# ebanalyse/ebnerd-benchmark

Hardware: AMD Instinct MI355X
Metric: training impressions/sec (higher is better)
Workload: dtype f32

## Files before the change

### ebnerd-benchmark_amd/csrc/ebn_attpool.hip

```cpp
#include "ebn_common.h"
#include "ebn_reduce.h"

namespace {

constexpr int POOL_THREADS = 256;
constexpr int POOL_WAVES = POOL_THREADS / 64;
constexpr float KERAS_EPS = 1e-7f;

__global__ __launch_bounds__(POOL_THREADS) void attpool_fwd_kernel(float* __restrict__ U,
                                                                    const float* __restrict__ b,
                                                                    const float* __restrict__ q,
                                                                    const float* __restrict__ X,
                                                                    float* __restrict__ out,
                                                                    float* __restrict__ w, int L, int E, int A) {
  extern __shared__ float sm[];
  const int64_t n = blockIdx.x;
  const int tid = threadIdx.x, lane = tid & 63, wave = tid >> 6;
  for (int l = wave; l < L; l += POOL_WAVES) {
    float* urow = U + (n * L + l) * A;
    float part = 0.f;
    for (int k = lane; k < A; k += 64) {
      const float u = tanhf(urow[k] + b[k]);
      urow[k] = u;
      part = fmaf(u, q[k], part);
// ... 40 lines not shown
    part = ebn_wave_sum(part);
    if (lane == 0) sm[l] = part;
  }
  __syncthreads();
  if (wave == 0) {
    float s = 0.f;
    for (int l = lane; l < L; l += 64) s = fmaf(w[n * L + l], sm[l], s);
    s = ebn_wave_sum(s);
    for (int l = lane; l < L; l += 64) de[n * L + l] = w[n * L + l] * (sm[l] - s);
  }
  if (dX == nullptr) return;
  for (int l = 0; l < L; ++l) {
    const float wl = w[n * L + l];
    float* dr = dX + (n * L + l) * E;
    for (int c = tid; c < E; c += POOL_THREADS) dr[c] = wl * g[c];
  }
}

constexpr int POOL_RB = 8;

__device__ __forceinline__ float4 ld4_clamped(const float* __restrict__ base, int64_t off, bool ok) {
  return *reinterpret_cast<const float4*>(base + (ok ? off : 0));
}
__device__ __forceinline__ float4 ld4_or_zero(const float* __restrict__ base, int64_t off, bool ok) {
  const float4 v = ld4_clamped(base, off, ok);
  float4 r;
  r.x = ok ? v.x : 0.f;
  r.y = ok ? v.y : 0.f;
  r.z = ok ? v.z : 0.f;
  r.w = ok ? v.w : 0.f;
  return r;
}

__global__ __launch_bounds__(POOL_THREADS) void attpool_fwd_vec_kernel(float* __restrict__ U,
                                                                        const float* __restrict__ b,
                                                                        const float* __restrict__ q,
                                                                        const float* __restrict__ X,
                                                                        float* __restrict__ out,
                                                                        float* __restrict__ w, int L, int E, int A) {
  extern __shared__ float sm[];
  __shared__ float4 part_acc[POOL_THREADS];
  const int64_t n = blockIdx.x;
  const int tid = threadIdx.x, lane = tid & 63, wave = tid >> 6;
  const int A4 = A >> 2, E4 = E >> 2;
  {
    const bool kok = lane < A4;
    const float4 bb = ld4_or_zero(b, lane * 4, kok), qq = ld4_or_zero(q, lane * 4, kok);
    for (int l0 = wave; l0 < L; l0 += POOL_WAVES * POOL_RB) {
      float4 u[POOL_RB];
#pragma unroll
      for (int j = 0; j < POOL_RB; ++j) {
        const int l = l0 + POOL_WAVES * j;
        u[j] = ld4_clamped(U, (n * L + l) * A + lane * 4, kok && l < L);
      }
#pragma unroll
      for (int j = 0; j < POOL_RB; ++j) {
        const int l = l0 + POOL_WAVES * j;
        if (l >= L) break;
        float4 t;
        t.x = tanhf(u[j].x + bb.x);
        t.y = tanhf(u[j].y + bb.y);
        t.z = tanhf(u[j].z + bb.z);
        t.w = tanhf(u[j].w + bb.w);
        if (kok) *reinterpret_cast<float4*>(U + (n * L + l) * A + lane * 4) = t;
        float part = kok ? fmaf(t.w, qq.w, fmaf(t.z, qq.z, fmaf(t.y, qq.y, t.x * qq.x))) : 0.f;
        part = ebn_wave_sum(part);
        if (lane == 0) sm[l] = part;
      }
    }
  }
  __syncthreads();
  if (wave == 0) {
    float s = 0.f;
    for (int l = lane; l < L; l += 64) {
      const float a = expf(sm[l]);
      sm[l] = a;
      s += a;
    }
    s = ebn_wave_sum(s) + KERAS_EPS;
    for (int l = lane; l < L; l += 64) {
      const float wl = sm[l] / s;
      sm[l] = wl;
      w[n * L + l] = wl;
    }
  }
  __syncthreads();
  const int NP = (E4 <= POOL_THREADS) ? POOL_THREADS / E4 : 1;
  for (int c0 = 0; c0 < E4; c0 += POOL_THREADS) {
    const int c4 = c0 + tid % ((E4 <= POOL_THREADS) ? E4 : POOL_THREADS);
    const int part = (E4 <= POOL_THREADS) ? tid / E4 : 0;
    const bool ok = c4 < E4 && part < NP;
    float4 acc = make_float4(0.f, 0.f, 0.f, 0.f);
    for (int l0 = part; l0 < L; l0 += NP * POOL_RB) {
      float4 x[POOL_RB];
#pragma unroll
      for (int j = 0; j < POOL_RB; ++j) {
        const int l = l0 + NP * j;
        x[j] = ld4_clamped(X, (n * L + l) * E + c4 * 4, ok && l < L);
      }
#pragma unroll
      for (int j = 0; j < POOL_RB; ++j) {
        const int l = l0 + NP * j;
        const float wl = (l < L) ? sm[l] : 0.f;
        acc.x = fmaf(wl, x[j].x, acc.x);
        acc.y = fmaf(wl, x[j].y, acc.y);
        acc.z = fmaf(wl, x[j].z, acc.z);
        acc.w = fmaf(wl, x[j].w, acc.w);
      }
    }
    if (NP > 1) {
      part_acc[tid] = acc;
      __syncthreads();
      if (part == 0 && ok) {
        for (int pp = 1; pp < NP; ++pp) {
          const float4 o = part_acc[pp * E4 + c4];
          acc.x += o.x;
          acc.y += o.y;
          acc.z += o.z;
          acc.w += o.w;
        }
      }
      __syncthreads();
    }
    if (part == 0 && ok) *reinterpret_cast<float4*>(out + n * E + c4 * 4) = acc;
  }
}

__global__ __launch_bounds__(POOL_THREADS) void attpool_bwd_pool_vec_kernel(const float* __restrict__ X,
                                                                             const float* __restrict__ w,
                                                                             const float* __restrict__ dout,
                                                                             float* __restrict__ dX,
                                                                             float* __restrict__ de, int L, int E,
                                                                             int write_dx) {
  extern __shared__ float sm[];
  const int64_t n = blockIdx.x;
  const int tid = threadIdx.x, lane = tid & 63, wave = tid >> 6;
  const int E4 = E >> 2;
  const float* g = dout + n * E;
  constexpr int VL = 4;
  float4 gg[VL];
#pragma unroll
  for (int v = 0; v < VL; ++v) gg[v] = ld4_or_zero(g, (lane + 64 * v) * 4, lane + 64 * v < E4);
  for (int l0 = wave; l0 < L; l0 += POOL_WAVES * POOL_RB) {
    float part[POOL_RB];
#pragma unroll
    for (int j = 0; j < POOL_RB; ++j) part[j] = 0.f;
#pragma unroll
    for (int v = 0; v < VL; ++v) {
      if (64 * v >= E4) break;
      float4 x[POOL_RB];
#pragma unroll
      for (int j = 0; j < POOL_RB; ++j) {
        const int l = l0 + POOL_WAVES * j;
        x[j] = ld4_clamped(X, (n * L + l) * E + (lane + 64 * v) * 4, l < L && lane + 64 * v < E4);
      }
#pragma unroll
      for (int j = 0; j < POOL_RB; ++j)
        part[j] = fmaf(gg[v].w, x[j].w, fmaf(gg[v].z, x[j].z, fmaf(gg[v].y, x[j].y, fmaf(gg[v].x, x[j].x, part[j]))));
    }
#pragma unroll
    for (int j = 0; j < POOL_RB; ++j) {
      const int l = l0 + POOL_WAVES * j;
      const float t = ebn_wave_sum(part[j]);
      if (lane == 0 && l < L) sm[l] = t;
    }
  }
  __syncthreads();
  if (wave == 0) {
    float s = 0.f;
    for (int l = lane; l < L; l += 64) s = fmaf(w[n * L + l], sm[l], s);
    s = ebn_wave_sum(s);
    for (int l = lane; l < L; l += 64) de[n * L + l] = w[n * L + l] * (sm[l] - s);
  }
  if (!write_dx) return;
  for (int c4 = tid; c4 < E4; c4 += POOL_THREADS) {
    const float4 gv = *reinterpret_cast<const float4*>(g + c4 * 4);
    for (int l = 0; l < L; ++l) {
      const float wl = w[n * L + l];
      *reinterpret_cast<float4*>(dX + (n * L + l) * E + c4 * 4) = make_float4(wl * gv.x, wl * gv.y, wl * gv.z, wl * gv.w);
    }
  }
}

__global__ __launch_bounds__(POOL_THREADS) void attpool_bwd_dpre_kernel(float* __restrict__ U,
                                                                         const float* __restrict__ q,
                                                                         const float* __restrict__ de,
                                                                         float* __restrict__ partials,
                                                                         int64_t R, int A, int64_t rpb) {
  const int64_t r0 = static_cast<int64_t>(blockIdx.x) * rpb;
  const int64_t r1 = (r0 + rpb < R) ? r0 + rpb : R;
  for (int k = threadIdx.x; k < A; k += POOL_THREADS) {
    const float qk = q[k];
    float dq = 0.f, db = 0.f;
    for (int64_t rb = r0; rb < r1; rb += 8) {
      float u[8], der[8];
#pragma unroll
      for (int j = 0; j < 8; ++j) {
        const int64_t r = (rb + j < r1) ? rb + j : r1 - 1;
        u[j] = U[r * A + k];
        der[j] = de[r];
      }
#pragma unroll
      for (int j = 0; j < 8; ++j) {
        if (rb + j >= r1) break;
        dq = fmaf(der[j], u[j], dq);
// ... 45 lines not shown
        *reinterpret_cast<float4*>(U + r * A + c4 * 4) = dp;
        db.x += dp.x;
        db.y += dp.y;
        db.z += dp.z;
        db.w += dp.w;
      }
    }
    *reinterpret_cast<float4*>(&sm[rs * A + c4 * 4]) = dq;
    *reinterpret_cast<float4*>(&sm[(RS + rs) * A + c4 * 4]) = db;
  }
  __syncthreads();
  for (int k = tid; k < A; k += POOL_THREADS) {
    float tq = 0.f, tb = 0.f;
    for (int i = 0; i < RS; ++i) {
      tq += sm[i * A + k];
      tb += sm[(RS + i) * A + k];
    }
    partials[(static_cast<int64_t>(blockIdx.x) * 2 + 0) * A + k] = tq;
    partials[(static_cast<int64_t>(blockIdx.x) * 2 + 1) * A + k] = tb;
  }
}

extern "C" int64_t ebn_attpool_partials_len(int64_t R, int32_t A) { return ebn_dim_ok(R, A) ? ebn_colred_blocks(R) * 2 * A : 0; }

extern "C" int ebn_attpool_fwd_f32(float* U, const float* b, const float* q, const float* X, float* out,
                                   float* w, int64_t n_seq, int32_t L, int32_t E, int32_t A,
                                   ebn_stream_t stream) {
  EBN_REQUIRE(U && b && q && X && out && w, EBN_ERR_BAD_ARG);
  EBN_REQUIRE(n_seq >= 0 && L > 0 && E > 0 && A > 0, EBN_ERR_BAD_ARG);
  EBN_REQUIRE(L <= 8192, EBN_ERR_UNSUPPORTED);
  if (n_seq == 0) return EBN_OK;
  const bool vec = (A % 4 == 0) && A <= 256 && (E % 4 == 0) && E <= 1024 && ebn_aligned16(U) && ebn_aligned16(b) &&
                   ebn_aligned16(q) && ebn_aligned16(X) && ebn_aligned16(out);
  if (vec)
    EBN_LAUNCH(attpool_fwd_vec_kernel, dim3(static_cast<unsigned>(n_seq)), dim3(POOL_THREADS),
                       L * sizeof(float), ebn_stream(stream), U, b, q, X, out, w, L, E, A);
  else
    EBN_LAUNCH(attpool_fwd_kernel, dim3(static_cast<unsigned>(n_seq)), dim3(POOL_THREADS),
                       L * sizeof(float), ebn_stream(stream), U, b, q, X, out, w, L, E, A);
  EBN_CHECK_LAUNCH();
  return EBN_OK;
}

extern "C" int ebn_attpool_bwd_pool_f32(const float* X, const float* w, const float* dout, float* dX,
                                        float* de, int64_t n_seq, int32_t L, int32_t E,
                                        ebn_stream_t stream) {
  EBN_REQUIRE(X && w && dout && de, EBN_ERR_BAD_ARG);
  EBN_REQUIRE(n_seq >= 0 && L > 0 && E > 0, EBN_ERR_BAD_ARG);
  EBN_REQUIRE(L <= 8192, EBN_ERR_UNSUPPORTED);
  if (n_seq == 0) return EBN_OK;
  const bool vec = (E % 4 == 0) && E <= 1024 && ebn_aligned16(X) && ebn_aligned16(dout) && ebn_aligned16(dX);
  if (vec)
    EBN_LAUNCH(attpool_bwd_pool_vec_kernel, dim3(static_cast<unsigned>(n_seq)), dim3(POOL_THREADS),
                       L * sizeof(float), ebn_stream(stream), X, w, dout, dX, de, L, E, dX != nullptr ? 1 : 0);
  else
    EBN_LAUNCH(attpool_bwd_pool_kernel, dim3(static_cast<unsigned>(n_seq)), dim3(POOL_THREADS),
                       L * sizeof(float), ebn_stream(stream), X, w, dout, dX, de, L, E);
  EBN_CHECK_LAUNCH();
  return EBN_OK;
}

extern "C" int ebn_attpool_bwd_dpre_f32(float* U, const float* q, const float* de, float* dq, float* db,
                                        float* partials, int64_t R, int32_t A, int32_t accumulate,
                                        ebn_stream_t stream) {
  EBN_REQUIRE(U && q && de && partials && ((dq != nullptr) == (db != nullptr)), EBN_ERR_BAD_ARG);
  EBN_REQUIRE(R >= 0 && A > 0, EBN_ERR_BAD_ARG);
  if (R == 0) return EBN_OK;
  const int64_t nb = ebn_colred_blocks(R);
  const int64_t rpb = ebn_ceil_div(R, nb);
  if ((A % 4) == 0 && A >= 4 && A <= 1024 && ebn_aligned16(U) && ebn_aligned16(q)) {
    const size_t lds = static_cast<size_t>(2) * (POOL_THREADS / (A / 4)) * A * sizeof(float);
    EBN_LAUNCH(attpool_bwd_dpre_vec_kernel, dim3(static_cast<unsigned>(nb)), dim3(POOL_THREADS), lds, ebn_stream(stream), U, q, de, partials,
                       R, A, rpb);
  } else {
    EBN_LAUNCH(attpool_bwd_dpre_kernel, dim3(static_cast<unsigned>(nb)), dim3(POOL_THREADS), 0,
                       ebn_stream(stream), U, q, de, partials, R, A, rpb);
  }
  EBN_CHECK_LAUNCH();
  if (dq == nullptr) return EBN_OK;
  ebn_reduce_partials(partials, nb, 2, A, 1.0f, dq, db, accumulate, nullptr, nullptr, ebn_stream(stream));
  EBN_CHECK_LAUNCH();
  return EBN_OK;
}
```

### ebnerd-benchmark_amd/csrc/ebn_gemm.hip

```cpp
#include <stdlib.h>

#include "ebn_common.h"
#include "ebn_finish.h"
#include "ebn_tn_finale.h"

typedef float ebn_f32x4 __attribute__((ext_vector_type(4)));
typedef int ebn_i32x4 __attribute__((ext_vector_type(4)));
__device__ ebn_f32x4 ebn_raw_buffer_load_x4(ebn_i32x4 rsrc, int voffset, int soffset, int aux) __asm("llvm.amdgcn.raw.buffer.load.v4f32");
__device__ void ebn_raw_buffer_load_lds(ebn_i32x4 rsrc, __attribute__((address_space(3))) void* lds, int size, int voffset,
                                        int soffset, int offset, int aux) __asm("llvm.amdgcn.raw.buffer.load.lds");

int ebn_gemm_direct_tn_slices(int64_t M, int64_t N, int64_t K);
int ebn_gemm_direct_tn_launch(int64_t M, int64_t N, int64_t K, float alpha, const float* A, int64_t lda, const float* B, int64_t ldb,
                              float* part, hipStream_t s);
bool ebn_gemm_direct_wanted(int32_t transA, int32_t transB, int64_t M, int64_t N, int64_t K);
int ebn_gemm_direct_launch(int32_t transB, int64_t M, int64_t N, int64_t K, float alpha, const float* A, int64_t lda, const float* B,
                           int64_t ldb, float* C, int64_t ldc, hipStream_t s);

namespace {

typedef float f32x16 __attribute__((ext_vector_type(16)));


typedef float f32x4n __attribute__((ext_vector_type(4)));
__device__ __forceinline__ float4 gload4(const __attribute__((address_space(1))) float* p) {
  const f32x4n t = *reinterpret_cast<const __attribute__((address_space(1))) f32x4n*>(p);
  return make_float4(t.x, t.y, t.z, t.w);
}
typedef ebn_i32x4 i32x4n;
__device__ __forceinline__ i32x4n make_rsrc(const float* base) {
  const unsigned long long a = reinterpret_cast<unsigned long long>(base);
  i32x4n r;
  r.x = static_cast<int>(static_cast<uint32_t>(a));
// ... 633 lines not shown
#pragma unroll
  for (int r = 0; r < 4; ++r) {
    const int64_t row = m0 + wm * 16 + 4 * kq + r;
    if (row >= M) continue;
    float v = alpha * acc[r];
    if (beta != 0.f) v += beta * C[row * ldc + col];
    if (epi.rs != nullptr)
      v = fmaf(epi.rs[row], epi.cv[static_cast<int64_t>(static_cast<uint32_t>(row) / static_cast<uint32_t>(epi.L)) * epi.ldcv + col], v);
    if (epi.bias != nullptr) v = fmaxf(v + epi.bias[col], 0.f);
    C[row * ldc + col] = v;
  }
}

template <bool KC, int T>
__device__ __forceinline__ void small_store_t(float* __restrict__ S, const float4 (&r)[SBK / T], int tid) {
  constexpr int THREADS = T * T / 4;
#pragma unroll
  for (int i = 0; i < SBK / T; ++i) {
    const int v = tid + i * THREADS;
    if (KC) {
      const int row = v / (SBK / 4);
      *reinterpret_cast<float4*>(&S[row * SLV + (((v % (SBK / 4)) * 4) ^ (((row >> 2) & 7) << 2))]) = r[i];
    } else {
      const int m4 = (v % (T / 4)) * 4;
      const int k = (v / (T / 4)) ^ (((m4 >> 2) & 7) << 2);
      S[(m4 + 0) * SLV + k] = r[i].x;
      S[(m4 + 1) * SLV + k] = r[i].y;
      S[(m4 + 2) * SLV + k] = r[i].z;
      S[(m4 + 3) * SLV + k] = r[i].w;
    }
  }
}

template <bool TA, bool TB, int T, bool FIN = false>
__device__ __forceinline__ void small_vec_body(int64_t M, int64_t N, int64_t K, float alpha, const float* __restrict__ A,
                                               int64_t lda, const float* __restrict__ B, int64_t ldb, float beta,
                                               float* __restrict__ C, int64_t ldc, GemmEpi epi, int64_t tile_x, int64_t tile_y,
                                               const EbnTnFinale* fin = nullptr) {
  extern __shared__ __attribute__((aligned(16))) float smem_small[];
  constexpr int THREADS = T * T / 4, SPT = SBK / T, WPR = T / 16;
  const int tid = threadIdx.x, lane = tid & 63, wave = tid >> 6;
  const int wm = wave / WPR, wn = wave % WPR;
  const int64_t m0 = tile_y * T, n0 = tile_x * T;
  const int nk = static_cast<int>((K + SBK - 1) / SBK), nk_full = static_cast<int>(K / SBK);
  constexpr int TILE = T * SLV;
  constexpr bool A_KC = !TA, B_KC = TB;
  const i32x4n arsrc = make_rsrc(A_KC ? A + m0 * lda : A + m0), brsrc = make_rsrc(B_KC ? B + n0 * ldb : B + n0);
  const uint32_t step_a = static_cast<uint32_t>((A_KC ? SBK : SBK * lda) * 4), step_b = static_cast<uint32_t>((B_KC ? SBK : SBK * ldb) * 4);
  uint32_t oa[SPT], ob[SPT];
#pragma unroll
  for (int i = 0; i < SPT; ++i) {
    const int v = tid + i * THREADS;
    if (A_KC) {
      int64_t r = m0 + v / (SBK / 4);
      r = r < M ? r : M - 1;
      oa[i] = static_cast<uint32_t>(((r - m0) * lda + (v % (SBK / 4)) * 4) * 4);
    } else {
      int64_t c = m0 + (v % (T / 4)) * 4;
      c = c + 3 < M ? c : M - 4;
      oa[i] = static_cast<uint32_t>(((v / (T / 4)) * lda + (c - m0)) * 4);
    }
    if (B_KC) {
      int64_t r = n0 + v / (SBK / 4);
      r = r < N ? r : N - 1;
      ob[i] = static_cast<uint32_t>(((r - n0) * ldb + (v % (SBK / 4)) * 4) * 4);
    } else {
      int64_t c = n0 + (v % (T / 4)) * 4;
      c = c + 3 < N ? c : N - 4;
      ob[i] = static_cast<uint32_t>(((v / (T / 4)) * ldb + (c - n0)) * 4);
    }
  }
  f32x4 acc0 = {0.f, 0.f, 0.f, 0.f}, acc1 = acc0, acc2 = acc0, acc3 = acc0;
// ... 57 lines not shown
  do {                                                                                                              \
    const float* ap__ = smem_small + (BUF) * 2 * TILE + (wm * 16 + r16) * SLV;                                      \
    const float* bp__ = smem_small + (BUF) * 2 * TILE + TILE + (wn * 16 + r16) * SLV;                               \
    float4 fa__[2][2], fb__[2][2];                                                                                  \
    if ((KT) < nk_full) {                                                                                           \
      EBN_SM_READ(0, 0);                                                                                            \
      EBN_SM_READ(1, 1);                                                                                            \
      __builtin_amdgcn_sched_barrier(0);      \
      EBN_SM_MUL(0);                                                                                                \
      __builtin_amdgcn_sched_barrier(0);                                                                            \
      EBN_SM_READ(0, 2);                                                                                            \
      __builtin_amdgcn_sched_barrier(0);                                                                            \
      EBN_SM_MUL(1);                                                                                                \
      __builtin_amdgcn_sched_barrier(0);                                                                            \
      EBN_SM_READ(1, 3);                                                                                            \
      __builtin_amdgcn_sched_barrier(0);                                                                            \
      EBN_SM_MUL(0);                                                                                                \
      EBN_SM_MUL(1);                                                                                                \
    } else {                                                                                                        \
      const int groups__ = static_cast<int>((K - static_cast<int64_t>(KT) * SBK + 31) / 32);                        \
      for (int g = 0; g < groups__; ++g) {                                                                          \
        EBN_SM_READ(0, g);                                                                                          \
        EBN_SM_MUL(0);                                                                                              \
      }                                                                                                             \
    }                                                                                                               \
  } while (0)
  EBN_SM_LOAD(0, 0);
  if (nk > 1) EBN_SM_LOAD(1, 1);
  EBN_SM_STORE(0, 0);
  __syncthreads();
  for (int kt = 0; kt < nk; kt += 2) {
    if (kt + 2 < nk) EBN_SM_LOAD(0, kt + 2);
    EBN_SM_MMA(0, kt);
    if (kt + 1 < nk) EBN_SM_STORE(1, 1);
    __syncthreads();
    if (kt + 1 >= nk) break;
    if (kt + 3 < nk) EBN_SM_LOAD(1, kt + 3);
    EBN_SM_MMA(1, kt + 1);
    if (kt + 2 < nk) EBN_SM_STORE(0, 0);
    __syncthreads();
  }
#undef EBN_SM_LOAD
#undef EBN_SM_STORE
#undef EBN_SM_MMA
#undef EBN_SM_READ
#undef EBN_SM_MUL
  const f32x4 acc = (acc0 + acc1) + (acc2 + acc3);
  if (do_colsum) {
    constexpr int CG = T / 4, KR = THREADS / CG;
    float* sc = smem_small;
    *reinterpret_cast<float4*>(&sc[(tid / CG) * (T + 4) + (tid % CG) * 4]) = csum;
    __syncthreads();
    if (tid < T && n0 + tid < N) {
      float t = 0.f;
      for (int r = 0; r < KR; ++r) t += sc[r * (T + 4) + tid];
      epi.colsum[n0 + tid] = t;
      if (FIN) ebn_adam_flat_apply(fin->adam, fin->adam.st->adam_alpha, (epi.colsum + n0 + tid) - fin->adam.grad, t);
    }
  }
  const int64_t col = n0 + wn * 16 + r16;
  if (col < N) {
    const float al = FIN ? fin->adam.st->adam_alpha : 0.f;
#pragma unroll
    for (int r = 0; r < 4; ++r) {
      const int64_t row = m0 + wm * 16 + 4 * kq + r;
      if (row >= M) continue;
      float v = alpha * acc[r];
      if (beta != 0.f) v += beta * C[row * ldc + col];
      if (epi.rs != nullptr)
        v = fmaf(epi.rs[row], epi.cv[static_cast<int64_t>(static_cast<uint32_t>(row) / static_cast<uint32_t>(epi.L)) * epi.ldcv + col], v);
      if (epi.bias != nullptr) v = fmaxf(v + epi.bias[col], 0.f);
      if (epi.l2w != nullptr) v = fmaf(epi.two_lambda, epi.l2w[row * ldc + col], v);
      C[row * ldc + col] = v;
      if (FIN) ebn_adam_flat_apply(fin->adam, al, (C + row * ldc + col) - fin->adam.grad, v);
    }
  }
}

template <bool TA, bool TB, int T>
__global__ __launch_bounds__(T * T / 4) void gemm_small_vec_kernel(int64_t M, int64_t N, int64_t K, float alpha,
                                                                      const float* __restrict__ A, int64_t lda,
                                                                      const float* __restrict__ B, int64_t ldb, float beta,
                                                                      float* __restrict__ C, int64_t ldc, GemmEpi epi) {
  small_vec_body<TA, TB, T>(M, N, K, alpha, A, lda, B, ldb, beta, C, ldc, epi, blockIdx.x, blockIdx.y);
}

struct SmallProblem {
  int64_t M, N, K;
  float alpha;
  const float* A;
  int64_t lda;
  const float* B;
  int64_t ldb;
  float beta;
  float* C;
  int64_t ldc;
  int32_t tiles_x, tiles;
};

__global__ __launch_bounds__(GEMM_THREADS) void gemm_small_pair_kernel(SmallProblem p0, SmallProblem p1) {
  const GemmEpi none{nullptr, nullptr, 0, 1, nullptr};
  const int b = blockIdx.x;
  if (b < p0.tiles)
    small_vec_body<true, false, 32>(p0.M, p0.N, p0.K, p0.alpha, p0.A, p0.lda, p0.B, p0.ldb, p0.beta, p0.C, p0.ldc, none,
                                    b % p0.tiles_x, b / p0.tiles_x);
  else
    small_vec_body<false, true, 32>(p1.M, p1.N, p1.K, p1.alpha, p1.A, p1.lda, p1.B, p1.ldb, p1.beta, p1.C, p1.ldc, none,
                                    (b - p0.tiles) % p1.tiles_x, (b - p0.tiles) / p1.tiles_x);
}

struct SmallGroup {
  SmallProblem p[EBN_TN_GROUP_MAX];
  float* colsum[EBN_TN_GROUP_MAX];
  const float* l2w[EBN_TN_GROUP_MAX];
  float two_lambda[EBN_TN_GROUP_MAX];
  int32_t first[EBN_TN_GROUP_MAX + 1];
  int32_t n;
// ... 47 lines not shown
    const int64_t per = (f.rest_total + nwg - 1) / nwg, e0 = static_cast<int64_t>(b) * per;
    const int64_t e1 = e0 + per < f.rest_total ? e0 + per : f.rest_total;
    for (int64_t e = e0 + tid; e < e1; e += NT) {
      int64_t off = e;
      int r = 0;
      while (r + 1 < f.n_rest && off >= f.rest_len[r]) off -= f.rest_len[r++];
      off += f.rest_off[r];
      ebn_adam_flat_apply(f.adam, al, off, f.adam.grad[off]);
    }
  }
  const int nh = (2 * f.A + 255) / 256 + 1;
  if (f.head_partials != nullptr && b < nh) {
    __syncthreads();
    ebn_user_head_finish_body(smem_small, b, nh, f.head_partials, f.B, f.A, f.dq, f.db, f.loss_rows, f.loss_out);
    if (b < nh - 1) {
      const int idx = b * 256 + tid;
      if (tid < 256 && idx < 2 * f.A) {
        const int sidx = idx / f.A, k = idx - sidx * f.A;
        float* gp = (sidx == 0 ? f.dq : f.db) + k;
        ebn_adam_flat_apply(f.adam, al, gp - f.adam.grad, *gp);
      }
    } else if (tid == 0 && f.n_l2 > 0) {
      float tot = 0.f;
      for (int l = 0; l < f.n_l2; ++l) {
        float tl = 0.f;
        for (int j = 0; j < f.l2_tiles[l]; ++j) tl += f.l2_part[l * f.l2_slots + j];
        tot += tl;
      }
      f.loss_out[0] += f.l2 * tot;
    }
  }
}

int launch_gemm_small(int transA, int transB, int64_t M, int64_t N, int64_t K, float alpha, const float* A, int64_t lda,
                      const float* B, int64_t ldb, float beta, float* C, int64_t ldc, int vecA, int vecB, hipStream_t s,
                      GemmEpi epi) {
  const dim3 grid(static_cast<unsigned>(ebn_ceil_div(N, SBN)), static_cast<unsigned>(ebn_ceil_div(M, SBM))), block(GEMM_THREADS);
  constexpr size_t lds = static_cast<size_t>(2) * 2 * SBM * SLD * sizeof(float);
#define EBN_SMALL_ONE(TA, TB, VA, VB)                                                                                     \
  do {                                                                                                                     \
    static const hipError_t attr__ = hipFuncSetAttribute(reinterpret_cast<const void*>(&gemm_small_kernel<TA, TB, VA, VB>), \
                                                         hipFuncAttributeMaxDynamicSharedMemorySize, static_cast<int>(lds)); \
    if (attr__ != hipSuccess) return static_cast<int>(attr__);                                                            \
    EBN_LAUNCH((gemm_small_kernel<TA, TB, VA, VB>), grid, block, lds, s, M, N, K, alpha, A, lda, B, ldb, beta, C, ldc, epi); \
  } while (0)
#define EBN_SMALL_VEC_T(TA, TB, T)                                                                                         \
  do {                                                                                                                     \
    constexpr size_t lds_t = static_cast<size_t>(2) * 2 * (T) * SLV * sizeof(float);                                       \
    static const hipError_t attr__ = hipFuncSetAttribute(reinterpret_cast<const void*>(&gemm_small_vec_kernel<TA, TB, T>), \
                                                         hipFuncAttributeMaxDynamicSharedMemorySize, static_cast<int>(lds_t)); \
    if (attr__ != hipSuccess) return static_cast<int>(attr__);                                                            \
    const dim3 grid_t(static_cast<unsigned>(ebn_ceil_div(N, T)), static_cast<unsigned>(ebn_ceil_div(M, T)));               \
    EBN_LAUNCH((gemm_small_vec_kernel<TA, TB, T>), grid_t, dim3((T) * (T) / 4), lds_t, s, M, N, K, alpha, A, lda, B, ldb, \
                       beta, C, ldc, epi);                                                                                 \
  } while (0)
#define EBN_SMALL_VEC(TA, TB) EBN_SMALL_VEC_T(TA, TB, 32)
  const bool fits32 = (K + SBK) * (transA ? lda : 1) * 4 + 64 * lda * 4 < (int64_t{1} << 31) &&
                      (K + SBK) * (transB ? 1 : ldb) * 4 + 64 * ldb * 4 < (int64_t{1} << 31);
#define EBN_SMALL(TA, TB)                              \
  do {                                                 \
    if (vecA && vecB && fits32) EBN_SMALL_VEC(TA, TB); \
    else EBN_SMALL_ONE(TA, TB, false, false);          \
  } while (0)
  if (!transA && !transB) EBN_SMALL(false, false);
  else if (!transA && transB) EBN_SMALL(false, true);
  else if (transA && !transB) EBN_SMALL(true, false);
  else EBN_SMALL(true, true);
#undef EBN_SMALL
#undef EBN_SMALL_VEC
#undef EBN_SMALL_VEC_T
#undef EBN_SMALL_ONE
  EBN_CHECK_LAUNCH();
  return EBN_OK;
}

}

struct GemmPlan {
  int bm, bn;
  int splits;
  int64_t kps;
  double cost;
};

static GemmPlan gemm_plan(int64_t M, int64_t N, int64_t K, int64_t ws_floats) {
  int64_t max_split = K / (4 * BK);
  if (max_split > 64) max_split = 64;
  const int64_t max_by_ws = (M * N > 0) ? ws_floats / (M * N) : 0;
  if (max_split > max_by_ws) max_split = max_by_ws;
  if (max_split < 1 || M * N >= (static_cast<int64_t>(1) << 31)) max_split = 1;
  static const struct {
    int bm, bn;
    double ts_full, ts_lone;
    int resident;
    int family;
  } kTiles[4] = {{128, 128, 1.15, 1.5, 3, 128}, {256, 64, 1.17, 1.5, 3, 256}, {64, 64, 0.32, 0.48, 4, 64}, {128, 64, 0.60, 0.8, 3, 96}};
  const double out_mb = static_cast<double>(M) * static_cast<double>(N) * 4e-6;
  GemmPlan best{128, 128, 1, ebn_ceil_div(K > 0 ? K : 1, BK) * BK, 1e300};
  {
    const int64_t wgs = ebn_ceil_div(M, SBM) * ebn_ceil_div(N, SBN);
    const int64_t tiles64 = ebn_ceil_div(M, 64) * ebn_ceil_div(N, 64);
    if (tiles64 <= 256 && K <= 4096) {
// ... 16 lines not shown
      if (sp == prev_s) continue;
      prev_s = sp;
      const int64_t W = ebn_ceil_div(tiles * sp, 256);
      const double full = static_cast<double>(W) * kTiles[t].ts_full;
      const double lone = static_cast<double>(ebn_ceil_div(W, kTiles[t].resident)) * kTiles[t].ts_lone;
      double cost = static_cast<double>(kps / BK) * (full > lone ? full : lone) + 3.0;
      if (sp > 1) cost += 4.5 + static_cast<double>(sp + 1) * out_mb / 2.5;
      if (kTiles[t].bm == 64 && sp > 1 && kps / BK >= 64 && W <= 6) cost *= 1.0 - 0.01 * static_cast<double>(W);
      if (cost < best.cost) best = GemmPlan{kTiles[t].bm, kTiles[t].bn, static_cast<int>(sp), kps, cost};
    }
  }
  return best;
}

extern "C" int64_t ebn_gemm_workspace_floats(int64_t M, int64_t N, int64_t K) {
  if (!ebn_dim_ok(M, N, K)) return 0;
  const GemmPlan p = gemm_plan(M, N, K, INT64_MAX / 4);
  int64_t slices = p.splits > 1 ? p.splits : 0;
  const int64_t tn = ebn_gemm_direct_tn_slices(M, N, K);
  if (tn > slices) slices = tn;
  return ebn_sat_mul(slices * M, N);
}

extern "C" int ebn_gemm_plan(int64_t M, int64_t N, int64_t K, int64_t workspace_floats, int32_t* bm, int32_t* bn,
                             int32_t* splits) {
  EBN_REQUIRE(M >= 0 && N >= 0 && K >= 0 && bm && bn && splits, EBN_ERR_BAD_ARG);
  const GemmPlan p = gemm_plan(M, N, K, workspace_floats);
  *bm = p.bm;
  *bn = p.bn;
  *splits = p.splits;
  return EBN_OK;
}

static int gemm_dispatch(int32_t transA, int32_t transB, int64_t M, int64_t N, int64_t K, float alpha, const float* A,
                         int64_t lda, const float* B, int64_t ldb, float beta, float* C, int64_t ldc, float* workspace,
                         int64_t workspace_floats, int32_t site, GemmEpi epi, hipStream_t s, int32_t* defer_parts = nullptr) {
  if (defer_parts != nullptr) {
    C = workspace;
    ldc = N;
    beta = 0.f;
    *defer_parts = 1;
  }
  const bool spanA = (transA ? (K + 16) * lda + 256 : 256 * lda + K + 16) * 4 < (int64_t{1} << 32);
  const bool spanB = (transB ? 256 * ldb + K + 16 : (K + 16) * ldb + 256) * 4 < (int64_t{1} << 32);
  const int vecA = ((lda % 4) == 0 && ebn_aligned16(A) && ((transA ? M : K) % 4) == 0 && spanA) ? 1 : 0;
  const int vecB = ((ldb % 4) == 0 && ebn_aligned16(B) && ((transB ? K : N) % 4) == 0 && spanB) ? 1 : 0;
  if ((epi.bias != nullptr || epi.rs != nullptr) && !(vecA && vecB)) return EBN_ERR_UNSUPPORTED;
  if (epi.bias == nullptr && epi.rs == nullptr && beta == 0.f && vecA && (vecB || !transB) &&
      ebn_gemm_direct_wanted(transA, transB, M, N, K)) {
    const int rc_dir = ebn_gemm_direct_launch(transB, M, N, K, alpha, A, lda, B, ldb, C, ldc, s);
    if (rc_dir != EBN_ERR_UNSUPPORTED) return rc_dir;
  }
  if (transA && !transB && epi.bias == nullptr && epi.rs == nullptr && workspace != nullptr &&
      M * N < (int64_t{1} << 31)) {
    const int z = ebn_gemm_direct_tn_slices(M, N, K);
    if (z >= 2 && workspace_floats >= static_cast<int64_t>(z) * M * N) {
      const int rc_tn = ebn_gemm_direct_tn_launch(M, N, K, alpha, A, lda, B, ldb, workspace, s);
      if (rc_tn == EBN_OK) {
        if (defer_parts != nullptr) {
          *defer_parts = z;
          return EBN_OK;
        }
        int64_t grid = ebn_ceil_div(M * N, 256);
        if (grid > 4096) grid = 4096;
        EBN_LAUNCH(splitk_reduce_kernel, dim3(static_cast<unsigned>(grid)), dim3(256), 0, s, workspace, z, M, N, beta, C, ldc, epi);
        EBN_CHECK_LAUNCH();
// ... 120 lines not shown
    const int rr = ebn_bias_relu_f32(C + r * ldc, bias, C + r * ldc, 1, static_cast<int32_t>(N), stream);
    if (rr != EBN_OK) return rr;
  }
  return (ldc == N) ? ebn_bias_relu_f32(C, bias, C, M, static_cast<int32_t>(N), stream) : EBN_OK;
}

extern "C" int ebn_gemm_f32_ws(int32_t transA, int32_t transB, int64_t M, int64_t N, int64_t K, float alpha,
                               const float* A, int64_t lda, const float* B, int64_t ldb, float beta,
                               float* C, int64_t ldc, float* workspace, int64_t workspace_floats,
                               ebn_stream_t stream) {
  return ebn_gemm_f32_site(transA, transB, M, N, K, alpha, A, lda, B, ldb, beta, C, ldc, workspace, workspace_floats, 0,
                           stream);
}

extern "C" int ebn_dense_bwd_pair_f32(int64_t R, int64_t K_in, int64_t N_out, const float* X, int64_t ldx, const float* dY,
                                      int64_t lddy, const float* W, int64_t ldw, float beta_w, float* dW, int64_t lddw,
                                      float* dX, int64_t lddx, float* workspace, int64_t workspace_floats,
                                      ebn_stream_t stream) {
  EBN_REQUIRE(R >= 0 && K_in >= 0 && N_out >= 0, EBN_ERR_BAD_ARG);
  if (K_in == 0 || N_out == 0) return EBN_OK;
  EBN_REQUIRE(X && dY && W && dW && dX, EBN_ERR_BAD_ARG);
  EBN_REQUIRE(ldx >= K_in && lddy >= N_out && ldw >= N_out && lddw >= N_out && lddx >= K_in, EBN_ERR_BAD_ARG);
  hipStream_t s = ebn_stream(stream);
  const bool aligned = (ldx % 4) == 0 && (lddy % 4) == 0 && (ldw % 4) == 0 && ebn_aligned16(X) && ebn_aligned16(dY) &&
                       ebn_aligned16(W) && (K_in % 4) == 0 && (N_out % 4) == 0;
  const int64_t span = (R + SBK) * (ldx > lddy ? ldx : lddy) * 4 + 64 * ((ldx > lddy ? ldx : lddy) > ldw ? (ldx > lddy ? ldx : lddy) : ldw) * 4;
  const bool small = R > 0 && gemm_plan(K_in, N_out, R, workspace ? workspace_floats : 0).bm == 32 &&
                     gemm_plan(R, K_in, N_out, workspace ? workspace_floats : 0).bm == 32;
  if (aligned && small && span < (int64_t{1} << 31)) {
    SmallProblem p0{K_in, N_out, R, 1.0f, X, ldx, dY, lddy, beta_w, dW, lddw, static_cast<int32_t>(ebn_ceil_div(N_out, SBN)), 0};
    p0.tiles = p0.tiles_x * static_cast<int32_t>(ebn_ceil_div(K_in, SBM));
    SmallProblem p1{R, K_in, N_out, 1.0f, dY, lddy, W, ldw, 0.0f, dX, lddx, static_cast<int32_t>(ebn_ceil_div(K_in, SBN)), 0};
    p1.tiles = p1.tiles_x * static_cast<int32_t>(ebn_ceil_div(R, SBM));
    constexpr size_t lds = static_cast<size_t>(2) * 2 * SBM * SLV * sizeof(float);
    static const hipError_t attr = hipFuncSetAttribute(reinterpret_cast<const void*>(&gemm_small_pair_kernel),
                                                       hipFuncAttributeMaxDynamicSharedMemorySize, static_cast<int>(lds));
    if (attr != hipSuccess) return static_cast<int>(attr);
    EBN_LAUNCH(gemm_small_pair_kernel, dim3(static_cast<unsigned>(p0.tiles + p1.tiles)), dim3(GEMM_THREADS), lds, s, p0, p1);
    EBN_CHECK_LAUNCH();
    return EBN_OK;
  }
  const GemmEpi none{nullptr, nullptr, 0, 1, nullptr};
  if (R == 0) {
    return gemm_dispatch(1, 0, K_in, N_out, 0, 1.0f, X, ldx, dY, lddy, beta_w, dW, lddw, workspace, workspace_floats, 0, none, s);
  }
  const int rc = gemm_dispatch(1, 0, K_in, N_out, R, 1.0f, X, ldx, dY, lddy, beta_w, dW, lddw, workspace, workspace_floats, 0, none, s);
  if (rc != EBN_OK) return rc;
  return gemm_dispatch(0, 1, R, K_in, N_out, 1.0f, dY, lddy, W, ldw, 0.0f, dX, lddx, workspace, workspace_floats, 0, none, s);
}

extern "C" int ebn_gemm_f32_rowmap(const int32_t* ids, int64_t table_rows, int64_t M, int64_t N, int64_t K, const float* table,
                                   int64_t ldt, const float* B, int64_t ldb, float* C, int64_t ldc, int32_t* oob_flag, ebn_stream_t stream) {
  EBN_REQUIRE(ebn_dim_ok(M, N, K) && table_rows > 0, EBN_ERR_BAD_ARG);
  if (M == 0 || N == 0) return EBN_OK;
  EBN_REQUIRE(ids && table && B && C && ldt >= K && ldb >= N && ldc >= N && K > 0, EBN_ERR_BAD_ARG);
  const bool ok = M >= 256 && (ldt % 4) == 0 && (ldb % 4) == 0 && (K % 4) == 0 && (N % 4) == 0 && ebn_aligned16(table) && ebn_aligned16(B) &&
                  (table_rows * ldt + K + 16) * 4 < (int64_t{1} << 32) && ((K + 16) * ldb + 256) * 4 < (int64_t{1} << 32);
  if (!ok) return EBN_ERR_UNSUPPORTED;
  GemmEpi epi{nullptr, nullptr, 0, 1, nullptr};
  epi.rowmap = ids;
  epi.rowmap_rows = table_rows;
  epi.oob = oob_flag;
  return launch_gemm<256, 64, 4>(0, 0, M, N, K, 1.0f, table, ldt, B, ldb, 0.0f, C, ldc, 1, 1, 1, ebn_ceil_div(K, BK) * BK, nullptr,
                                 ebn_stream(stream), 0, epi);
}

extern "C" int ebn_gemm_tn_group_f32(const ebn_tn_problem* problems, int32_t n, ebn_stream_t stream) {
  EBN_REQUIRE(problems != nullptr && n >= 1 && n <= EBN_TN_GROUP_MAX, EBN_ERR_BAD_ARG);
  int64_t tiles64 = 0;
  for (int i = 0; i < n; ++i) {
    const ebn_tn_problem& q = problems[i];
// ... 96 lines not shown
```

### include/ebnerd_hip.h

```cpp
#ifndef EBNERD_HIP_H
#define EBNERD_HIP_H

#include <stdint.h>

#ifdef __cplusplus
extern "C" {
#endif

#define EBN_ABI_VERSION 1

#define EBN_OK 0
#define EBN_ERR_BAD_ARG (-1)
#define EBN_ERR_UNSUPPORTED (-2)
#define EBN_ERR_ALIGN (-3)

typedef void* ebn_stream_t;

#define EBN_SITE_NEWS_IN 0
#define EBN_SITE_NEWS_ATT 1
#define EBN_SITE_MLP0 8
#define EBN_N_SITES 12

typedef struct ebn_step_state {
  uint32_t step;
// ... 30 lines not shown
                                            float drop_p, int32_t* range_flag, ebn_stream_t stream);
int ebn_fixed_to_f32(int64_t* acc, float* out, int64_t n, int32_t* range_flag, ebn_stream_t stream);
int ebn_adam_keras_step_fixed_f32(float* theta, int64_t* acc, float* m, float* v, int64_t n, const ebn_step_state* st,
                                  double beta1, double beta2, double eps, float grad_scale, int32_t* range_flag,
                                  ebn_stream_t stream);

int64_t ebn_gemm_split_workspace_bytes(int64_t M, int64_t N, int64_t K);
int ebn_gemm_f32_split(int32_t transA, int32_t transB, int64_t M, int64_t N, int64_t K, float alpha, const float* A,
                       int64_t lda, const float* B, int64_t ldb, float beta, float* C, int64_t ldc, void* workspace,
                       int64_t workspace_bytes, ebn_stream_t stream);
int64_t ebn_planes_bytes(int64_t rows, int64_t K);
int ebn_split_planes_f32(const float* src, int64_t ld, int64_t rows, int64_t K, int32_t trans, void* planes,
                         ebn_stream_t stream);
int ebn_gather_split_planes_f32(const int32_t* ids, const float* table, int64_t n_rows, int32_t D, int64_t V,
                                const ebn_step_state* st, int32_t site, float drop_p, int32_t* oob_flag, void* planes_n,
                                void* planes_t, ebn_stream_t stream);
int64_t ebn_gemm_planes_workspace_floats(int64_t M, int64_t N, int64_t K);
int ebn_gemm_planes_f32(const void* a_planes, int64_t M, const void* b_planes, int64_t N, int64_t K, float alpha, float beta,
                        float* C, int64_t ldc, float* workspace, int64_t workspace_floats, ebn_stream_t stream);
int64_t ebn_gemm_prec_workspace_bytes(int64_t M, int64_t N, int64_t K, int32_t precision);
int ebn_gemm_f32_prec(int32_t transA, int32_t transB, int64_t M, int64_t N, int64_t K, float alpha, const float* A,
                      int64_t lda, const float* B, int64_t ldb, float beta, float* C, int64_t ldc, void* workspace,
                      int64_t workspace_bytes, int32_t precision, ebn_stream_t stream);

int64_t ebn_shard_plan_workspace_ints(int64_t V, int32_t world);
int ebn_shard_plan_i32(const int32_t* ids, int64_t n_tok, int64_t V, int32_t world, int32_t cyclic, int64_t cap,
                       int32_t* workspace, int32_t* slot_rows, int32_t* inv, int32_t* counts, ebn_stream_t stream);

int ebn_gemm_f32(int32_t transA, int32_t transB, int64_t M, int64_t N, int64_t K, float alpha,
                 const float* A, int64_t lda, const float* B, int64_t ldb, float beta, float* C,
                 int64_t ldc, ebn_stream_t stream);
int64_t ebn_gemm_workspace_floats(int64_t M, int64_t N, int64_t K);
int ebn_gemm_plan(int64_t M, int64_t N, int64_t K, int64_t workspace_floats, int32_t* bm, int32_t* bn, int32_t* splits);
int ebn_gemm_f32_ws(int32_t transA, int32_t transB, int64_t M, int64_t N, int64_t K, float alpha,
                    const float* A, int64_t lda, const float* B, int64_t ldb, float beta, float* C,
                    int64_t ldc, float* workspace, int64_t workspace_floats, ebn_stream_t stream);

int64_t ebn_gemm_partials_workspace_floats(int64_t M, int64_t N, int64_t K);
int ebn_gemm_f32_partials(int32_t transA, int32_t transB, int64_t M, int64_t N, int64_t K, float alpha, const float* A,
                          int64_t lda, const float* B, int64_t ldb, float* workspace, int64_t workspace_floats,
                          int32_t* n_parts, ebn_stream_t stream);

#define EBN_FINISH_SPLITK 0
#define EBN_FINISH_COLRED 1
#define EBN_FINISH_HEAD 2
#define EBN_FINISH_MAX_JOBS 6
typedef struct {
  int32_t kind;
  int32_t n_parts;
  int64_t rows, cols;
  const float* partials;
  float* out0;
  float* out1;
  int64_t ld;
  float beta, scale;
  const float* loss_rows;
  float* loss_out;
} ebn_finish_job;
int ebn_grad_finish_f32(const ebn_finish_job* jobs, int32_t n_jobs, ebn_stream_t stream);

#define EBN_ADAM_FLAT_MAX_REST 12
typedef struct ebn_adam_flat {
  float* theta;
  const float* grad;
  float* m;
  float* v;
// ... 481 lines not shown
```

Before: 25820.

## Prefetch attention-pool inputs early and add single-buffer three-block small GEMM form

The forward attention-pool kernel is templated so the first U rows and a batch of X rows are prefetched into registers before and during the tanh/score phase, overlapping the weighted-sum loads with the softmax. Backward pooling gets a VL template (2 for E<=512) with hoisted X loads and weight reads. Separately, the small GEMM gains a single-LDS-buffer variant that lets three workgroups sit on a CU, picked when the tile count makes three slots per CU need fewer waves. This trades extra register pressure and extra syncs for better latency hiding and occupancy, and adds tuning hooks and an env override.

```diff
diff --git a/ebnerd-benchmark_amd/csrc/ebn_attpool.hip b/ebnerd-benchmark_amd/csrc/ebn_attpool.hip
--- a/ebnerd-benchmark_amd/csrc/ebn_attpool.hip
+++ b/ebnerd-benchmark_amd/csrc/ebn_attpool.hip
@@ -96,26 +96,45 @@
   return r;
 }
 
-__global__ __launch_bounds__(POOL_THREADS) void attpool_fwd_vec_kernel(float* __restrict__ U,
-                                                                        const float* __restrict__ b,
-                                                                        const float* __restrict__ q,
-                                                                        const float* __restrict__ X,
-                                                                        float* __restrict__ out,
-                                                                        float* __restrict__ w, int L, int E, int A) {
+template <int PFA, int PFB, int MIN_WAVES>
+__global__ __launch_bounds__(POOL_THREADS, MIN_WAVES) void attpool_fwd_vec_kernel(float* __restrict__ U,
+                                                                                   const float* __restrict__ b,
+                                                                                   const float* __restrict__ q,
+                                                                                   const float* __restrict__ X,
+                                                                                   float* __restrict__ out,
+                                                                                   float* __restrict__ w, int L, int E, int A) {
   extern __shared__ float sm[];
   __shared__ float4 part_acc[POOL_THREADS];
   const int64_t n = blockIdx.x;
   const int tid = threadIdx.x, lane = tid & 63, wave = tid >> 6;
   const int A4 = A >> 2, E4 = E >> 2;
+  const int NP = POOL_THREADS / E4, c4 = tid % E4, part = tid / E4;
+  const bool ok = part < NP;
+  constexpr int PF = PFA + PFB;
+  float4 xp[PF];
   {
     const bool kok = lane < A4;
-    const float4 bb = ld4_or_zero(b, lane * 4, kok), qq = ld4_or_zero(q, lane * 4, kok);
+    const float4 bb = ld4_clamped(b, lane * 4, kok), qq = ld4_clamped(q, lane * 4, kok);
+    float4 u[POOL_RB];
+#pragma unroll
+    for (int j = 0; j < POOL_RB; ++j) {
+      const int l = wave + POOL_WAVES * j;
+      u[j] = ld4_clamped(U, (n * L + l) * A + lane * 4, kok && l < L);
+    }
+    __builtin_amdgcn_sched_barrier(0);
+#pragma unroll
+    for (int j = 0; j < PFA; ++j) {
+      const int l = part + NP * j;
+      xp[j] = ld4_clamped(X, (n * L + l) * E + c4 * 4, ok && l < L);
+    }
+    __builtin_amdgcn_sched_barrier(0);
     for (int l0 = wave; l0 < L; l0 += POOL_WAVES * POOL_RB) {
-      float4 u[POOL_RB];
-#pragma unroll
-      for (int j = 0; j < POOL_RB; ++j) {
-        const int l = l0 + POOL_WAVES * j;
-        u[j] = ld4_clamped(U, (n * L + l) * A + lane * 4, kok && l < L);
+      if (l0 != wave) {
+#pragma unroll
+        for (int j = 0; j < POOL_RB; ++j) {
+          const int l = l0 + POOL_WAVES * j;
+          u[j] = ld4_clamped(U, (n * L + l) * A + lane * 4, kok && l < L);
+        }
       }
 #pragma unroll
       for (int j = 0; j < POOL_RB; ++j) {
@@ -132,6 +151,11 @@
         if (lane == 0) sm[l] = part;
       }
     }
+#pragma unroll
+    for (int j = PFA; j < PF; ++j) {
+      const int l = part + NP * j;
+      xp[j] = ld4_clamped(X, (n * L + l) * E + c4 * 4, ok && l < L);
+    }
   }
   __syncthreads();
   if (wave == 0) {
@@ -149,13 +173,19 @@
     }
   }
   __syncthreads();
-  const int NP = (E4 <= POOL_THREADS) ? POOL_THREADS / E4 : 1;
-  for (int c0 = 0; c0 < E4; c0 += POOL_THREADS) {
-    const int c4 = c0 + tid % ((E4 <= POOL_THREADS) ? E4 : POOL_THREADS);
-    const int part = (E4 <= POOL_THREADS) ? tid / E4 : 0;
-    const bool ok = c4 < E4 && part < NP;
+  {
     float4 acc = make_float4(0.f, 0.f, 0.f, 0.f);
-    for (int l0 = part; l0 < L; l0 += NP * POOL_RB) {
+#pragma unroll
+    for (int j = 0; j < PF; ++j) {
+      const int l = part + NP * j;
+      const bool in = l < L;
+      const float wl = in ? sm[l] : 0.f;
+      acc.x = fmaf(wl, in ? xp[j].x : 0.f, acc.x);
+      acc.y = fmaf(wl, in ? xp[j].y : 0.f, acc.y);
+      acc.z = fmaf(wl, in ? xp[j].z : 0.f, acc.z);
+      acc.w = fmaf(wl, in ? xp[j].w : 0.f, acc.w);
+    }
+    for (int l0 = part + NP * PF; l0 < L; l0 += NP * POOL_RB) {
       float4 x[POOL_RB];
 #pragma unroll
       for (int j = 0; j < POOL_RB; ++j) {
@@ -190,6 +220,7 @@
   }
 }
 
+template <int VL>
 __global__ __launch_bounds__(POOL_THREADS) void attpool_bwd_pool_vec_kernel(const float* __restrict__ X,
                                                                              const float* __restrict__ w,
                                                                              const float* __restrict__ dout,
@@ -201,26 +232,32 @@
   const int tid = threadIdx.x, lane = tid & 63, wave = tid >> 6;
   const int E4 = E >> 2;
   const float* g = dout + n * E;
-  constexpr int VL = 4;
+#define EBN_POOL_LOAD_X(L0)                                                                                               \
+  _Pragma("unroll") for (int v = 0; v < VL; ++v) {                                                                        \
+    _Pragma("unroll") for (int j = 0; j < POOL_RB; ++j) {                                                                 \
+      const int l = (L0) + POOL_WAVES * j < L ? (L0) + POOL_WAVES * j : L - 1;                                            \
+      x[v][j] = *reinterpret_cast<const float4*>(X + (n * L + l) * E + (lane + 64 * v < E4 ? (lane + 64 * v) * 4 : 0));   \
+    }                                                                                                                     \
+  }
+  float4 x[VL][POOL_RB];
+  EBN_POOL_LOAD_X(wave);
+  __builtin_amdgcn_sched_barrier(0);
   float4 gg[VL];
 #pragma unroll
-  for (int v = 0; v < VL; ++v) gg[v] = ld4_or_zero(g, (lane + 64 * v) * 4, lane + 64 * v < E4);
+  for (int v = 0; v < VL; ++v) gg[v] = ld4_clamped(g, (lane + 64 * v) * 4, lane + 64 * v < E4);
+  const float w0 = w[n * L + (lane < L ? lane : 0)];
   for (int l0 = wave; l0 < L; l0 += POOL_WAVES * POOL_RB) {
+    if (l0 != wave) EBN_POOL_LOAD_X(l0);
     float part[POOL_RB];
 #pragma unroll
     for (int j = 0; j < POOL_RB; ++j) part[j] = 0.f;
 #pragma unroll
     for (int v = 0; v < VL; ++v) {
-      if (64 * v >= E4) break;
-      float4 x[POOL_RB];
-#pragma unroll
-      for (int j = 0; j < POOL_RB; ++j) {
-        const int l = l0 + POOL_WAVES * j;
-        x[j] = ld4_clamped(X, (n * L + l) * E + (lane + 64 * v) * 4, l < L && lane + 64 * v < E4);
-      }
+      const float m = lane + 64 * v < E4 ? 1.0f : 0.0f;
+      const float4 gv = make_float4(gg[v].x * m, gg[v].y * m, gg[v].z * m, gg[v].w * m);
 #pragma unroll
       for (int j = 0; j < POOL_RB; ++j)
-        part[j] = fmaf(gg[v].w, x[j].w, fmaf(gg[v].z, x[j].z, fmaf(gg[v].y, x[j].y, fmaf(gg[v].x, x[j].x, part[j]))));
+        part[j] = fmaf(gv.w, x[v][j].w, fmaf(gv.z, x[v][j].z, fmaf(gv.y, x[v][j].y, fmaf(gv.x, x[v][j].x, part[j]))));
     }
 #pragma unroll
     for (int j = 0; j < POOL_RB; ++j) {
@@ -229,12 +266,15 @@
       if (lane == 0 && l < L) sm[l] = t;
     }
   }
+#undef EBN_POOL_LOAD_X
   __syncthreads();
   if (wave == 0) {
     float s = 0.f;
-    for (int l = lane; l < L; l += 64) s = fmaf(w[n * L + l], sm[l], s);
+    if (lane < L) s = fmaf(w0, sm[lane], s);
+    for (int l = lane + 64; l < L; l += 64) s = fmaf(w[n * L + l], sm[l], s);
     s = ebn_wave_sum(s);
-    for (int l = lane; l < L; l += 64) de[n * L + l] = w[n * L + l] * (sm[l] - s);
+    if (lane < L) de[n * L + lane] = w0 * (sm[lane] - s);
+    for (int l = lane + 64; l < L; l += 64) de[n * L + l] = w[n * L + l] * (sm[l] - s);
   }
   if (!write_dx) return;
   for (int c4 = tid; c4 < E4; c4 += POOL_THREADS) {
@@ -346,8 +386,12 @@
   if (n_seq == 0) return EBN_OK;
   const bool vec = (A % 4 == 0) && A <= 256 && (E % 4 == 0) && E <= 1024 && ebn_aligned16(U) && ebn_aligned16(b) &&
                    ebn_aligned16(q) && ebn_aligned16(X) && ebn_aligned16(out);
-  if (vec)
-    EBN_LAUNCH(attpool_fwd_vec_kernel, dim3(static_cast<unsigned>(n_seq)), dim3(POOL_THREADS),
+  const int rows_per_part = vec ? ebn_ceil_div(L, POOL_THREADS / (E / 4)) : 0;
+  if (vec && rows_per_part > 16 && rows_per_part <= 26 && n_seq <= 512)
+    EBN_LAUNCH((attpool_fwd_vec_kernel<4, 22, 2>), dim3(static_cast<unsigned>(n_seq)), dim3(POOL_THREADS),
+                       L * sizeof(float), ebn_stream(stream), U, b, q, X, out, w, L, E, A);
+  else if (vec)
+    EBN_LAUNCH((attpool_fwd_vec_kernel<4, 12, 4>), dim3(static_cast<unsigned>(n_seq)), dim3(POOL_THREADS),
                        L * sizeof(float), ebn_stream(stream), U, b, q, X, out, w, L, E, A);
   else
     EBN_LAUNCH(attpool_fwd_kernel, dim3(static_cast<unsigned>(n_seq)), dim3(POOL_THREADS),
@@ -364,8 +408,11 @@
   EBN_REQUIRE(L <= 8192, EBN_ERR_UNSUPPORTED);
   if (n_seq == 0) return EBN_OK;
   const bool vec = (E % 4 == 0) && E <= 1024 && ebn_aligned16(X) && ebn_aligned16(dout) && ebn_aligned16(dX);
-  if (vec)
-    EBN_LAUNCH(attpool_bwd_pool_vec_kernel, dim3(static_cast<unsigned>(n_seq)), dim3(POOL_THREADS),
+  if (vec && E <= 512)
+    EBN_LAUNCH(attpool_bwd_pool_vec_kernel<2>, dim3(static_cast<unsigned>(n_seq)), dim3(POOL_THREADS),
+                       L * sizeof(float), ebn_stream(stream), X, w, dout, dX, de, L, E, dX != nullptr ? 1 : 0);
+  else if (vec)
+    EBN_LAUNCH(attpool_bwd_pool_vec_kernel<4>, dim3(static_cast<unsigned>(n_seq)), dim3(POOL_THREADS),
                        L * sizeof(float), ebn_stream(stream), X, w, dout, dX, de, L, E, dX != nullptr ? 1 : 0);
   else
     EBN_LAUNCH(attpool_bwd_pool_kernel, dim3(static_cast<unsigned>(n_seq)), dim3(POOL_THREADS),
diff --git a/ebnerd-benchmark_amd/csrc/ebn_gemm.hip b/ebnerd-benchmark_amd/csrc/ebn_gemm.hip
--- a/ebnerd-benchmark_amd/csrc/ebn_gemm.hip
+++ b/ebnerd-benchmark_amd/csrc/ebn_gemm.hip
@@ -1,4 +1,6 @@
 #include <stdlib.h>
+
+#include <atomic>
 
 #include "ebn_common.h"
 #include "ebn_finish.h"
@@ -698,12 +700,14 @@
   }
 }
 
-template <bool TA, bool TB, int T, bool FIN = false>
+template <bool TA, bool TB, int T, bool FIN = false, int NBUF = 2>
 __device__ __forceinline__ void small_vec_body(int64_t M, int64_t N, int64_t K, float alpha, const float* __restrict__ A,
                                                int64_t lda, const float* __restrict__ B, int64_t ldb, float beta,
                                                float* __restrict__ C, int64_t ldc, GemmEpi epi, int64_t tile_x, int64_t tile_y,
                                                const EbnTnFinale* fin = nullptr) {
   extern __shared__ __attribute__((aligned(16))) float smem_small[];
+  static_assert(NBUF == 1 || NBUF == 2, "one or two LDS buffers");
+  constexpr int B1 = NBUF - 1;
   constexpr int THREADS = T * T / 4, SPT = SBK / T, WPR = T / 16;
   const int tid = threadIdx.x, lane = tid & 63, wave = tid >> 6;
   const int wm = wave / WPR, wn = wave % WPR;
@@ -827,11 +831,13 @@
   for (int kt = 0; kt < nk; kt += 2) {
     if (kt + 2 < nk) EBN_SM_LOAD(0, kt + 2);
     EBN_SM_MMA(0, kt);
-    if (kt + 1 < nk) EBN_SM_STORE(1, 1);
+    if (NBUF == 1 && kt + 1 < nk) __syncthreads();
+    if (kt + 1 < nk) EBN_SM_STORE(1, B1);
     __syncthreads();
     if (kt + 1 >= nk) break;
     if (kt + 3 < nk) EBN_SM_LOAD(1, kt + 3);
-    EBN_SM_MMA(1, kt + 1);
+    EBN_SM_MMA(B1, kt + 1);
+    if (NBUF == 1 && kt + 2 < nk) __syncthreads();
     if (kt + 2 < nk) EBN_SM_STORE(0, 0);
     __syncthreads();
   }
@@ -878,6 +884,14 @@
                                                                       const float* __restrict__ B, int64_t ldb, float beta,
                                                                       float* __restrict__ C, int64_t ldc, GemmEpi epi) {
   small_vec_body<TA, TB, T>(M, N, K, alpha, A, lda, B, ldb, beta, C, ldc, epi, blockIdx.x, blockIdx.y);
+}
+
+template <bool TA, bool TB>
+__global__ __launch_bounds__(GEMM_THREADS, 3) void gemm_small_vec3_kernel(int64_t M, int64_t N, int64_t K, float alpha,
+                                                                           const float* __restrict__ A, int64_t lda,
+                                                                           const float* __restrict__ B, int64_t ldb, float beta,
+                                                                           float* __restrict__ C, int64_t ldc, GemmEpi epi) {
+  small_vec_body<TA, TB, 32, false, 1>(M, N, K, alpha, A, lda, B, ldb, beta, C, ldc, epi, blockIdx.x, blockIdx.y);
 }
 
 struct SmallProblem {
@@ -991,10 +1005,26 @@
   }
 }
 
+constexpr int64_t SMALL_SLOTS2 = 2 * 256, SMALL_SLOTS3 = 3 * 256;
+constexpr size_t SMALL_LDS2 = static_cast<size_t>(2) * 2 * SBM * SLV * sizeof(float), SMALL_LDS3 = SMALL_LDS2 / 2;
+static_assert(3 * SMALL_LDS3 <= 163840 && SMALL_LDS3 <= 54613, "three single-buffer workgroups per CU");
+std::atomic<int> g_small_form{[] {
+  const char* e = getenv("EBN_GEMM_SMALL_FORM");
+  const int f = e ? atoi(e) : 0;
+  return (f == 2 || f == 3) ? f : 0;
+}()};
+
+int small_form_for(int64_t tiles) {
+  const int forced = g_small_form.load(std::memory_order_relaxed);
+  if (forced != 0) return forced;
+  return (tiles > SMALL_SLOTS2 && ebn_ceil_div(tiles, SMALL_SLOTS3) < ebn_ceil_div(tiles, SMALL_SLOTS2)) ? 3 : 2;
+}
+
 int launch_gemm_small(int transA, int transB, int64_t M, int64_t N, int64_t K, float alpha, const float* A, int64_t lda,
                       const float* B, int64_t ldb, float beta, float* C, int64_t ldc, int vecA, int vecB, hipStream_t s,
                       GemmEpi epi) {
   const dim3 grid(static_cast<unsigned>(ebn_ceil_div(N, SBN)), static_cast<unsigned>(ebn_ceil_div(M, SBM))), block(GEMM_THREADS);
+  const bool form3 = small_form_for(static_cast<int64_t>(grid.x) * grid.y) == 3;
   constexpr size_t lds = static_cast<size_t>(2) * 2 * SBM * SLD * sizeof(float);
 #define EBN_SMALL_ONE(TA, TB, VA, VB)                                                                                     \
   do {                                                                                                                     \
@@ -1013,7 +1043,18 @@
     EBN_LAUNCH((gemm_small_vec_kernel<TA, TB, T>), grid_t, dim3((T) * (T) / 4), lds_t, s, M, N, K, alpha, A, lda, B, ldb, \
                        beta, C, ldc, epi);                                                                                 \
   } while (0)
-#define EBN_SMALL_VEC(TA, TB) EBN_SMALL_VEC_T(TA, TB, 32)
+#define EBN_SMALL_VEC3(TA, TB)                                                                                             \
+  do {                                                                                                                     \
+    static const hipError_t attr__ = hipFuncSetAttribute(reinterpret_cast<const void*>(&gemm_small_vec3_kernel<TA, TB>),   \
+                                                         hipFuncAttributeMaxDynamicSharedMemorySize, static_cast<int>(SMALL_LDS3)); \
+    if (attr__ != hipSuccess) return static_cast<int>(attr__);                                                            \
+    EBN_LAUNCH((gemm_small_vec3_kernel<TA, TB>), grid, block, SMALL_LDS3, s, M, N, K, alpha, A, lda, B, ldb, beta, C, ldc, epi); \
+  } while (0)
+#define EBN_SMALL_VEC(TA, TB)           \
+  do {                                  \
+    if (form3) EBN_SMALL_VEC3(TA, TB);  \
+    else EBN_SMALL_VEC_T(TA, TB, 32);   \
+  } while (0)
   const bool fits32 = (K + SBK) * (transA ? lda : 1) * 4 + 64 * lda * 4 < (int64_t{1} << 31) &&
                       (K + SBK) * (transB ? 1 : ldb) * 4 + 64 * ldb * 4 < (int64_t{1} << 31);
 #define EBN_SMALL(TA, TB)                              \
@@ -1027,6 +1068,7 @@
   else EBN_SMALL(true, true);
 #undef EBN_SMALL
 #undef EBN_SMALL_VEC
+#undef EBN_SMALL_VEC3
 #undef EBN_SMALL_VEC_T
 #undef EBN_SMALL_ONE
   EBN_CHECK_LAUNCH();
@@ -1109,6 +1151,26 @@
   return EBN_OK;
 }
 
+extern "C" int ebn_gemm_small_resident(int32_t form) {
+  if (form != 2 && form != 3) return 0;
+  const void* fn = form == 3 ? reinterpret_cast<const void*>(&gemm_small_vec3_kernel<false, false>)
+                             : reinterpret_cast<const void*>(&gemm_small_vec_kernel<false, false, 32>);
+  const size_t lds = form == 3 ? SMALL_LDS3 : SMALL_LDS2;
+  int blocks = 0;
+  if (hipFuncSetAttribute(fn, hipFuncAttributeMaxDynamicSharedMemorySize, static_cast<int>(lds)) != hipSuccess ||
+      hipOccupancyMaxActiveBlocksPerMultiprocessor(&blocks, fn, GEMM_THREADS, lds) != hipSuccess) {
+    (void)hipGetLastError();
+    return 0;
+  }
+  return blocks;
+}
+
+extern "C" int ebn_gemm_small_force_form(int32_t form) {
+  return g_small_form.exchange((form == 2 || form == 3) ? form : 0, std::memory_order_relaxed);
+}
+
+extern "C" int ebn_gemm_small_form(int64_t tiles) { return small_form_for(tiles); }
+
 static int gemm_dispatch(int32_t transA, int32_t transB, int64_t M, int64_t N, int64_t K, float alpha, const float* A,
                          int64_t lda, const float* B, int64_t ldb, float beta, float* C, int64_t ldc, float* workspace,
                          int64_t workspace_floats, int32_t site, GemmEpi epi, hipStream_t s, int32_t* defer_parts = nullptr) {
@@ -1295,11 +1357,10 @@
     p0.tiles = p0.tiles_x * static_cast<int32_t>(ebn_ceil_div(K_in, SBM));
     SmallProblem p1{R, K_in, N_out, 1.0f, dY, lddy, W, ldw, 0.0f, dX, lddx, static_cast<int32_t>(ebn_ceil_div(K_in, SBN)), 0};
     p1.tiles = p1.tiles_x * static_cast<int32_t>(ebn_ceil_div(R, SBM));
-    constexpr size_t lds = static_cast<size_t>(2) * 2 * SBM * SLV * sizeof(float);
     static const hipError_t attr = hipFuncSetAttribute(reinterpret_cast<const void*>(&gemm_small_pair_kernel),
-                                                       hipFuncAttributeMaxDynamicSharedMemorySize, static_cast<int>(lds));
+                                                       hipFuncAttributeMaxDynamicSharedMemorySize, static_cast<int>(SMALL_LDS2));
     if (attr != hipSuccess) return static_cast<int>(attr);
-    EBN_LAUNCH(gemm_small_pair_kernel, dim3(static_cast<unsigned>(p0.tiles + p1.tiles)), dim3(GEMM_THREADS), lds, s, p0, p1);
+    EBN_LAUNCH(gemm_small_pair_kernel, dim3(static_cast<unsigned>(p0.tiles + p1.tiles)), dim3(GEMM_THREADS), SMALL_LDS2, s, p0, p1);
     EBN_CHECK_LAUNCH();
     return EBN_OK;
   }
diff --git a/include/ebnerd_hip.h b/include/ebnerd_hip.h
--- a/include/ebnerd_hip.h
+++ b/include/ebnerd_hip.h
@@ -86,6 +86,9 @@
                  int64_t ldc, ebn_stream_t stream);
 int64_t ebn_gemm_workspace_floats(int64_t M, int64_t N, int64_t K);
 int ebn_gemm_plan(int64_t M, int64_t N, int64_t K, int64_t workspace_floats, int32_t* bm, int32_t* bn, int32_t* splits);
+int ebn_gemm_small_resident(int32_t form);
+int ebn_gemm_small_form(int64_t tiles);
+int ebn_gemm_small_force_form(int32_t form);
 int ebn_gemm_f32_ws(int32_t transA, int32_t transB, int64_t M, int64_t N, int64_t K, float alpha,
                     const float* A, int64_t lda, const float* B, int64_t ldb, float beta, float* C,
                     int64_t ldc, float* workspace, int64_t workspace_floats, ebn_stream_t stream);
```

Result: no change. 25860, median of 4 (+0.2%).
